# koide3/fast_gicp

Hardware: AMD Instinct MI355X
Metric: registrations/sec (100-iter reuse) + final fitness_score; achieved HBM GB/s (higher is better)
Workload: dtype f64

## Files before the change

### fast_gicp_amd/capi.py

```python
import ctypes as C
import os

import numpy as np

from . import build as _build

REG_NONE, REG_MIN_EIG, REG_NORMALIZED_MIN_EIG, REG_PLANE, REG_FROBENIUS = range(5)
DIRECT27, DIRECT7, DIRECT1, DIRECT_RADIUS = range(4)
NDT_P2D, NDT_D2D = 0, 1
COMPUTE_FP64, COMPUTE_FP32, COMPUTE_CUDA_COMPAT = 0, 1, 2
VOXEL_ADDITIVE, VOXEL_ADDITIVE_WEIGHTED, VOXEL_MULTIPLICATIVE = range(3)
VOXEL_NDT_SUMS = 3

EXPORTED_SYMBOLS = None


class LmParams(C.Structure):
    _fields_ = [("max_iterations", C.c_int), ("rotation_epsilon", C.c_double), ("transformation_epsilon", C.c_double), ("lm_max_iterations", C.c_int),
                ("lm_init_lambda_factor", C.c_double), ("optimizer", C.c_int)]


class LmResult(C.Structure):
    _fields_ = [("T", C.c_double * 16), ("H", C.c_double * 36), ("final_error", C.c_double), ("converged", C.c_int), ("nr_iterations", C.c_int),
                ("num_linearize", C.c_int), ("num_error_evals", C.c_int), ("lm_failed", C.c_int), ("num_launches", C.c_int)]


class EngineParams(C.Structure):
    _fields_ = [("struct_size", C.c_int), ("sort_mode", C.c_int), ("sort_items", C.c_int), ("sort_fused_bits", C.c_int), ("sort_two_pass_max", C.c_int),
                ("sort_coop_watchdog_ticks", C.c_ulonglong), ("knn_nearest_first_max_points", C.c_int), ("knn_block", C.c_int), ("coherent_min_points", C.c_int),
                ("bitmap_min_points", C.c_int), ("bitmap_max_bytes", C.c_ulonglong), ("persistent", C.c_int), ("persist_watchdog_ticks", C.c_ulonglong),
                ("peer_watchdog_ticks", C.c_ulonglong), ("lm_everywhere", C.c_int), ("cost_prio", C.c_int), ("cost_split", C.c_int), ("cost_group_max", C.c_int),
                ("cost_max_blocks", C.c_int), ("cost_target_items", C.c_longlong), ("zerocopy_result", C.c_int), ("host_wait_block", C.c_int),
                ("result_query_spins", C.c_ulonglong), ("side_stream", C.c_int), ("pinned_upload_max", C.c_ulonglong), ("zerocopy_upload_max", C.c_ulonglong),
                ("avg_fused", C.c_int), ("nn1_seed", C.c_int)]


def default_engine_params():
    p = EngineParams()
    load().fvh_default_engine_params(C.byref(p))
    return p


class FvhError(RuntimeError):
    pass


_LIB = None


# ... 356 lines not shown

def comm_unique_id():
    buf = (C.c_char * 128)()
    rc = load().fvh_comm_unique_id(buf)
    if rc != 0:
        raise FvhError("fvh_comm_unique_id failed: %d" % rc)
    return bytes(buf)


def debug_slot_pool(device=0):
    r, a, c = C.c_int(0), C.c_int(0), C.c_int(0)
    load().fvh_debug_slot_pool(int(device), C.byref(r), C.byref(a), C.byref(c))
    return r.value, a.value, c.value


def debug_sort_routes():
    a = (C.c_int * 4)()
    rc = load().fvh_debug_sort_routes(a)
    if rc != 0:
        raise FvhError("fvh_debug_sort_routes: status %d" % rc)
    return list(a)


def debug_xcd_local():
    w, a = C.c_int(0), C.c_int(0)
    load().fvh_debug_xcd_local(C.byref(w), C.byref(a))
    return w.value, a.value


LM_REPLAY_ARGTYPES = [C.c_int, C.c_void_p, C.c_void_p, C.c_int, C.c_void_p, C.c_void_p, C.c_void_p]
# ... 529 lines not shown
```

### fast_gicp_amd/csrc/fvh_capi.hip

```cpp
#include <hip/hip_runtime.h>
#include <dlfcn.h>

#include <algorithm>
#include <cmath>
#include <cstdio>
#include <cstdlib>
#include <atomic>
#include <chrono>
#include <cstring>
#include <functional>
#include <map>
#include <mutex>
#include <string>
#include <type_traits>
#include <unordered_map>
#include <vector>

#include "../../include/fast_vgicp_hip.h"
#include "kernels_compat.hpp"
#include "kernels_cost.hpp"
#include "kernels_cov.hpp"
#include "kernels_downsample.hpp"
#include "kernels_outlier.hpp"
#include "kernels_peer.hpp"
// ... 9 lines not shown
  int device = 0;
  fvh_engine_params params = env_engine_defaults();
  hipStream_t stream = nullptr;
  std::string err;
  int align_optimizer = 0;
  int precision = FVH_COMPUTE_FP64;
  bool float_cost() const { return precision != FVH_COMPUTE_FP64; }
  std::vector<int> offsets_host{0, 0, 0};
  int n_off = 1;
  DevBuf fit_best;
  DevBuf sort_coop;
  unsigned sort_seq = 0;
  DevBuf rbf_sums;
  bool abort_word_dirty = false;
  int last_persist_blocks = 0;
  bool zero_copy_armed = false;
  DevBuf bcast;
  unsigned long long persist_seq = 0;
  DevBuf offsets_dev, state, partials, ticket, corr, misc, fit, staging, sort_keys, sort_idx, sort_hist;
  void* pinned = nullptr;
  void* upload_pinned = nullptr;
  size_t upload_pinned_cap = 0;
  hipEvent_t upload_done[2] = {nullptr, nullptr};
  bool upload_busy[2] = {false, false};
  int upload_slot = 0;
  bool ensure_upload_pinned(size_t bytes) {
    if (bytes <= upload_pinned_cap) return true;
    for (int s = 0; s < 2; s++) {
      if (upload_busy[s]) { (void)hipEventSynchronize(upload_done[s]); upload_busy[s] = false; }
      if (!upload_done[s] && hipEventCreateWithFlags(&upload_done[s], hipEventDisableTiming) != hipSuccess) { (void)hipGetLastError(); return false; }
// ... 1040 lines not shown
}
int fvh_vgicp_set_lm_trace(fvh_vgicp* h, int on) { CHECK_HANDLE(h); return shared::set_lm_trace(h, on); }
int fvh_vgicp_get_lm_trace(fvh_vgicp* h, int* n, double* rows6) { CHECK_HANDLE(h); return shared::get_lm_trace(&h->e, n, rows6); }
int fvh_vgicp_fitness_score(fvh_vgicp* h, const double* T, double max_range, double* score) { CHECK_HANDLE(h); return do_fitness(&h->e, h->source, h->target, T, max_range, score); }
int fvh_vgicp_profile_enable(fvh_vgicp* h, int on) { CHECK_HANDLE_HOST_ONLY(h); return shared::profile_enable(h, on); }
int fvh_vgicp_profile_reset(fvh_vgicp* h) { CHECK_HANDLE(h); return shared::profile_reset(h); }
int fvh_vgicp_profile_get(fvh_vgicp* h, const char* cls, double* ms, int* n) { CHECK_HANDLE(h); return profile_get(&h->e, cls, ms, n); }
int fvh_vgicp_debug_set_voxel_hint(fvh_vgicp* h, int num_voxels) { CHECK_HANDLE(h); h->voxelmap.nv_hint = num_voxels; return FVH_OK; }
int fvh_vgicp_debug_get_persist_aborts(fvh_vgicp* h, int* n) { CHECK_HANDLE(h); if (!n) return FVH_ERR_INVALID_ARGUMENT; *n = h->e.persist_aborts; return FVH_OK; }
int fvh_vgicp_debug_get_persist_grid(fvh_vgicp* h, int* blocks, int* capacity) {
  CHECK_HANDLE(h);
  if (blocks) *blocks = h->e.last_persist_blocks;
  if (capacity) *capacity = persistent_capacity<MODE_VGICP>(&h->e);
  return FVH_OK;
}
int fvh_debug_sort_routes(int* counts4) {
  if (!counts4) return FVH_ERR_INVALID_ARGUMENT;
  for (int i = 0; i < 4; i++) counts4[i] = g_sort_routes[i].load();
  return FVH_OK;
}
int fvh_debug_xcd_local(int* wanted, int* placement_aborts) {
  if (wanted) *wanted = xcd_local_wanted() ? 1 : 0;
  if (placement_aborts) *placement_aborts = g_xcd_local_strikes.load();
  return FVH_OK;
}
int fvh_debug_slot_pool(int device, int* reserved, int* active, int* recent) {
  int r = 0, a = 0, c = 0;
  g_slots.snapshot(device, &r, &a, &c);
  if (reserved) *reserved = r;
  if (active) *active = a;
// ... 550 lines not shown
```

### fast_gicp_amd/csrc/host_runtime.inc.hpp

```cpp


constexpr int MAX_COST_BLOCKS = MAX_PARTIAL_ROWS;

struct DevBuf {
  void* p = nullptr;
  size_t cap = 0;
  hipError_t ensure(size_t bytes) {
    if (bytes <= cap) return hipSuccess;
    if (p) { hipError_t e = hipFree(p); p = nullptr; cap = 0; if (e != hipSuccess) return e; }
    size_t want = bytes + bytes / 4 + 256;
    hipError_t e = hipMalloc(&p, want);
    if (e == hipSuccess) cap = want;
    return e;
  }
  void release() { if (p) (void)hipFree(p); p = nullptr; cap = 0; }
  template <typename T> T* as() const { return reinterpret_cast<T*>(p); }
};

inline const char* fvh_env(const char* name) { return getenv(name); }
inline long long fvh_env_ll(const char* name, long long dflt) { const char* v = fvh_env(name); return v ? atoll(v) : dflt; }
inline unsigned long long fvh_env_ull(const char* name, unsigned long long dflt) { const char* v = fvh_env(name); return v ? strtoull(v, nullptr, 10) : dflt; }
constexpr int COHERENT_MIN_POINTS = 32768;
struct ProcessParams { int slot_max_split, contended_slot_pct, xcd_local, small_grid_layout; };
inline const ProcessParams& process_params() {
// ... 27 lines not shown
    p.peer_watchdog_ticks = fvh_env_ull("FVH_PEER_WATCHDOG_TICKS", 200'000'000ull);
    p.lm_everywhere = (int)fvh_env_ll("FVH_LM_EVERYWHERE", 1);
    { const char* v = fvh_env("FVH_COST_PRIO"); p.cost_prio = v ? (atoi(v) != 0 ? 1 : 0) : -1; }
    p.cost_split = (int)fvh_env_ll("FVH_COST_SPLIT", 1);
    p.cost_group_max = (int)std::min<long long>(std::max(1LL, fvh_env_ll("FVH_COST_GROUP_MAX", COST_CH)), COST_CH);
    { const long long b = fvh_env_ll("FVH_COST_MAX_BLOCKS", MAX_PARTIAL_ROWS); p.cost_max_blocks = (int)(b < 1 ? 1 : (b > MAX_PARTIAL_ROWS ? MAX_PARTIAL_ROWS : b)); }
    p.cost_target_items = fvh_env_ll("FVH_COST_TARGET_ITEMS", 256LL * 256 * 2);
    p.zerocopy_result = (int)fvh_env_ll("FVH_ZEROCOPY_RESULT", 1);
    { const char* v = fvh_env("FVH_HOST_WAIT"); p.host_wait_block = (v && std::string(v) == "block") ? 1 : 0; }
    p.result_query_spins = fvh_env_ull("FVH_RESULT_QUERY_SPINS", 1024ull);
    p.side_stream = fvh_env_ll("FVH_SIDE_STREAM", 1) != 0 ? 1 : 0;
    p.pinned_upload_max = fvh_env_ull("FVH_PINNED_UPLOAD_MAX", 8ull << 20);
    p.zerocopy_upload_max = fvh_env_ull("FVH_ZEROCOPY_UPLOAD_MAX", 1ull << 20);
    p.avg_fused = fvh_env_ll("FVH_AVG_FUSED", 1) != 0 ? 1 : 0;
    p.nn1_seed = fvh_env_ll("FVH_NN1_SEED", 1) != 0 ? 1 : 0;
    return p;
  }();
  return d;
}
inline const char* check_engine_params(const fvh_engine_params& p) {
  if (p.struct_size != (int)sizeof(fvh_engine_params)) return "engine params: struct_size does not match this library's fvh_engine_params (start from fvh_default_engine_params / fvh_*_get_engine_params)";
  if (p.sort_mode < 0 || p.sort_mode > 3) return "engine params: sort_mode must be 0..3";
  if (p.sort_fused_bits != 0 && p.sort_fused_bits != 9 && p.sort_fused_bits != 10) return "engine params: sort_fused_bits must be 0, 9 or 10";
  if (p.knn_block != 64 && p.knn_block != 128 && p.knn_block != 256) return "engine params: knn_block must be 64, 128 or 256";
  if (p.cost_group_max < 1 || p.cost_group_max > COST_CH) return "engine params: cost_group_max must be 1..4";
  if (p.cost_max_blocks < 1 || p.cost_max_blocks > MAX_PARTIAL_ROWS) return "engine params: cost_max_blocks must be 1..1024";
  if (p.cost_target_items < 1) return "engine params: cost_target_items must be positive";
  if (p.lm_everywhere < 0 || p.lm_everywhere > 2 || p.cost_prio < -1 || p.cost_prio > 1) return "engine params: lm_everywhere must be 0..2, cost_prio -1..1";
  if (p.bitmap_max_bytes > (16ull << 30)) return "engine params: bitmap_max_bytes beyond 16 GiB (the LM kernel indexes its words with 32 bits)";
  if (p.sort_items < 0 || p.sort_items > SORT_ITEMS_MAX || (p.sort_items & 63)) return "engine params: sort_items must be 0 or a multiple of 64 up to 1024";
  return nullptr;
}

struct CloudDev {
  int n = 0, k = 0;
  DevBuf box;
  DevBuf bbox2;
  DevBuf order;
  DevBuf pts, cov, nbr, bbox, sorted;
  bool has_pts = false, has_cov = false, has_nbr = false, has_sorted = false;
  DevBuf cov_sorted;
  bool has_cov_sorted = false;
  bool nbr_tile_only = false;
// ... 139 lines not shown
    reserved[dev] -= g.n;
    active[dev]--;
    if (recent[dev] > active[dev] + 1) {
      if (++calm[dev] >= DECAY_AFTER) { recent[dev]--; calm[dev] = 0; }
    } else {
      calm[dev] = 0;
    }
  }
};
SlotPool g_slots;
constexpr int XCD_LOCAL_MAX_STRIKES = 3;
std::atomic<int> g_xcd_local_strikes{0};
inline bool xcd_local_wanted() {
  return process_params().xcd_local && g_xcd_local_strikes.load() < XCD_LOCAL_MAX_STRIKES;
}
struct GridPlan { int nb = 0; int ng = 0; int local = 0; };
inline int small_grid_layout() {
  return process_params().small_grid_layout;
}
inline int default_groups(int nb) {
  if (nb > SINGLE_LEVEL_MAX_BLOCKS) return TICKET_GROUPS;
  return (small_grid_layout() == 2 && nb >= 2 * TICKET_GROUPS) ? TICKET_GROUPS : 1;
}
```

### fast_gicp_amd/csrc/host_stages.inc.hpp

```cpp

int upload_cloud(Engine* e, CloudDev& c, const float* xyz, int n, int stride, bool on_device, bool want_box = true ,
                 hipStream_t on = nullptr ) {
  hipStream_t const st = on ? on : e->stream;
  if (n < 0 || (n > 0 && !xyz)) return e->fail(FVH_ERR_INVALID_ARGUMENT, "set_cloud: null points");
  if (stride != 3 && stride != 4) return e->fail(FVH_ERR_INVALID_ARGUMENT, "set_cloud: stride must be 3 or 4 floats");
  HIP_OR_FAIL(e, c.pts.ensure(sizeof(float4) * (size_t)std::max(n, 1)));
  c.n = n;
  c.has_pts = true;
  c.has_sorted = false;
  if (n == 0) return FVH_OK;
  unsigned* boxp = nullptr;
  c.has_box = want_box;
  if (want_box) {
    const bool fresh_box = c.box.p == nullptr;
    HIP_OR_FAIL(e, c.box.ensure(64));
    if (fresh_box || c.box_dirty) HIP_OR_FAIL(e, hipMemsetAsync(c.box.p, 0, 64, st));
    c.box_dirty = true;
    boxp = c.box.as<unsigned>();
  }
  auto pack = [&](const float* srcp, int slot) -> int {
    pack_points_kernel<<<pack_grid(n, boxp != nullptr), 256, 0, st>>>(srcp, n, stride, c.pts.as<float4>(), boxp);
    HIP_OR_FAIL(e, hipGetLastError());
    if (slot >= 0) { HIP_OR_FAIL(e, hipEventRecord(e->upload_done[slot], st)); e->upload_busy[slot] = true; }
    return FVH_OK;
// ... 581 lines not shown
int persistent_capacity(Engine* e) {
  static std::mutex mu;
  static int cap[16][2];
  std::lock_guard<std::mutex> lk(mu);
  const int pi = e->float_cost() ? 1 : 0, dev = e->device & 15;
  if (cap[dev][pi] <= 0) {
    int per_cu = 0, cus = 0;
    hipError_t r = pi ? hipOccupancyMaxActiveBlocksPerMultiprocessor(&per_cu, cost_kernel<float, MODE, true>, 256, 0)
                      : hipOccupancyMaxActiveBlocksPerMultiprocessor(&per_cu, cost_kernel<double, MODE, true>, 256, 0);
    if (r != hipSuccess || hipDeviceGetAttribute(&cus, hipDeviceAttributeMultiprocessorCount, e->device) != hipSuccess) return 0;
    cap[dev][pi] = per_cu * cus;
  }
  return cap[dev][pi];
}

struct CostShape { int group, groups_per_src; long long n_walk; int blocks; int split; };
inline CostShape cost_shape(const Engine* e, const CostSource& src, int mode = MODE_VGICP, bool device_lm = false) {
  const long long target_items = e->params.cost_target_items;
  const int max_blocks = e->params.cost_max_blocks;
  const int group_max = e->params.cost_group_max;
  const int n_off = src.n_off_override > 0 ? src.n_off_override : e->n_off;
  CostShape s;
  const int n_expected = src.n_shape > 0 ? std::min(src.n_shape, src.n_upper) : src.n_upper;
  const int groups = (int)std::min<long long>(n_off, std::max<long long>((n_off + group_max - 1) / group_max, target_items / std::max(n_expected, 1)));
  s.group = (n_off + groups - 1) / groups;
  s.groups_per_src = (n_off + s.group - 1) / s.group;
  s.n_walk = n_expected;
  if (e->sharded() && src.shardable) { const Tile t = peer_tile(e, src.n_upper); s.n_walk = std::max(t.hi - t.lo, 0); }
  if (src.device_tile) s.n_walk = (n_expected + e->shard_ranks() - 1) / std::max(1, e->shard_ranks());
  s.blocks = (int)std::max<long long>(1, std::min<long long>(max_blocks, (s.n_walk * s.groups_per_src + 255) / 256));
// ... 73 lines not shown
    if (MODE == MODE_VGICP && e->peer.attached()) P.peer = e->peer.view(peer_xbase);
    P.peer_watchdog_ticks = e->params.peer_watchdog_ticks;
  }
  int blocks = shape.blocks;
  (void)n_walk;
  {
    int cap = persistent_capacity<MODE>(e);
    if (cap <= 0) return e->fail(FVH_ERR_HIP, "cost kernel: occupancy query failed");
    if (e->peer.attached()) cap = std::max(1, cap / std::max(1, e->peer.ranks_on_device));
    blocks = std::min(blocks, cap);
    if (plan && plan->nb > 0) blocks = std::min(blocks, plan->nb);
  }
  P.ng = (plan && plan->ng > 0) ? plan->ng : default_groups(blocks);
  if (P.ng > blocks) P.ng = 1;
  P.xcd_local = 0; P.lm_everywhere = 0;
  {
    const int prio = e->params.cost_prio;
    int cus = 256;
    (void)hipDeviceGetAttribute(&cus, hipDeviceAttributeMultiprocessorCount, e->device);
    P.prio_from = cus;
    P.prio_mode = prio >= 0 ? prio : ((persistent && blocks > cus && blocks <= 2 * cus) ? 1 : 0);
    const int everywhere = e->params.lm_everywhere;
    P.lm_everywhere = (persistent && P.ng > 1 && (everywhere == 2 || (everywhere == 1 && blocks <= 2 * cus))) ? 1 : 0;
  }
  if (persistent && plan) P.xcd_local = plan->local;
  GangParams G{blocks, nullptr};
  const int gangs = multi ? multi->k : 1;
  if (multi) {
    P.st = e->multi_state.as<LmState>(); P.partials = e->multi_partials.as<double>(); P.ticket = e->multi_ticket.as<unsigned>();
    P.bcast = e->multi_bcast.as<double>(); P.corr = e->multi_corr.as<int>(); P.lm_trace = nullptr;
    P.xcd_local = 0; P.prio_mode = 0;
    int cus = 256;
    (void)hipDeviceGetAttribute(&cus, hipDeviceAttributeMultiprocessorCount, e->device);
    P.lm_everywhere = (persistent && P.ng > 1 && (e->params.lm_everywhere == 2 || (e->params.lm_everywhere == 1 && (long long)gangs * blocks <= 2 * cus))) ? 1 : 0;
    G.guesses = e->multi_guess.as<PoseD>();
  }
  if (!multi && e->abort_word_dirty) {
    HIP_OR_FAIL(e, hipMemsetAsync(reinterpret_cast<char*>(e->state.p) + sizeof(LmState) - 8, 0, 8, e->stream));
    e->abort_word_dirty = false;
  }
  if (persistent) {
    P.watchdog_ticks = fvh_env_ull("FVH_PERSIST_WATCHDOG_TICKS", e->params.persist_watchdog_ticks);
    if (P.peer.n > 1 && P.watchdog_ticks) P.watchdog_ticks = std::max(P.watchdog_ticks, 2 * P.peer_watchdog_ticks);
    const int zc = e->params.zerocopy_result;
    P.result_host = (zc && (!e->prof.on || e->prof.cost_only)) ? (multi ? e->multi_result_dev : e->result_dev) : nullptr;
    e->zero_copy_armed = P.result_host != nullptr;
    if (!multi) P.bcast = e->bcast.as<double>();
    P.launch_tag = ++e->persist_seq;
    e->last_persist_blocks = blocks;
    (void)e->gang_begin(false);
  }
  {
    ProfScope ps(e, "cost");
    const bool gauss_newton = (host_phase < 0 ? e->align_optimizer : 0) != 0;
    by_flag(e->float_cost(), [&](auto f32) { by_flag(P.group == 1, [&](auto one) { by_flag(gauss_newton, [&](auto gn) { by_flag(persistent, [&](auto pers) {
      using Real = std::conditional_t<decltype(f32)::value, float, double>;
      constexpr int CH = decltype(one)::value ? 1 : COST_CH;
      if (multi) lm_gang_kernel<Real, MODE, decltype(pers)::value, CH, decltype(gn)::value><<<gangs * blocks, 256, 0, e->stream>>>(P, G);
      else cost_kernel<Real, MODE, decltype(pers)::value, CH, decltype(gn)::value><<<blocks, 256, 0, e->stream>>>(P);
    }); }); }); });
  }
  if (persistent) e->gang_end();
  HIP_OR_FAIL(e, hipGetLastError());
  return FVH_OK;
}

int allreduce_sums(Engine* e) {
  LmState* st = e->state.as<LmState>();
  int rc = g_rccl.AllReduce(st->sums, st->sums, PART_STRIDE,  8,  0, e->comm, e->stream);
  if (rc != 0) return e->fail(FVH_ERR_COMM, "ncclAllReduce failed with code " + std::to_string(rc));
  return FVH_OK;
}
// ... 146 lines not shown
  r->num_launches = (int)launches;
}

inline void leave_handle(Engine* e, const LmState& h, const fvh_lm_params& p, int corr_kind, int n_src) {
  e->prev_steps = e->last_steps;
  e->last_steps = p.optimizer ? std::max(1, (int)h.num_linearize) : 1 + h.num_error_evals;
  e->lin = h.x_lin;
  e->corr_sel = h.corr_cur;
  e->has_corr = true;
  e->corr_kind = corr_kind;
  e->corr_n_src = n_src;
}

template <int MODE>
int align_begin(Engine* e, AlignCtx& c, const CostSource& src, VoxelMapDev& vm, const double* guess16, const fvh_lm_params* params,
                bool retried = false, bool no_persist = false, const GridPlan* forced_plan = nullptr ) {
  hipEvent_t const fence = e->crowd_fence;
  e->crowd_fence = nullptr;
  e->lm_crowds_chip = false;
  if (!guess16) return e->fail(FVH_ERR_INVALID_ARGUMENT, "align: null argument");
  if (!vm.valid) return e->fail(FVH_ERR_BAD_STATE, "align: target voxel map not built");
  c = AlignCtx{};
  fvh_lm_params& p = c.p;
  if (params) p = *params; else fvh_default_lm_params(&p);
  std::memcpy(c.guess16, guess16, sizeof(c.guess16));
  e->align_optimizer = p.optimizer != 0 ? 1 : 0;
  c.retried = retried; c.no_persist = no_persist; c.grant_dev = e->device;
  HIP_OR_FAIL(e, e->corr.ensure(2 * sizeof(int) * (size_t)std::max(src.n_upper, 1) * e->n_off));
  const PoseD guess = pose_from_colmajor16(guess16);
  c.degenerate = p.max_iterations <= 0;
  if (c.degenerate) {
// ... 11 lines not shown
  if (c.persistent) {
    int cap = persistent_capacity<MODE>(e);
    if (e->peer.attached()) cap = std::max(1, cap / std::max(1, e->peer.ranks_on_device));
    const int want = std::min(cost_shape(e, src, MODE, true).blocks, std::max(cap, 1));
    const bool local_ok = xcd_local_wanted();
    c.grant = g_slots.acquire(e->device, std::max(cap, 1), want);
    int granted = c.grant.n;
    if (granted <= 0) {
      if (c.sharded) granted = want;
      else c.persistent = false;
    }
    c.plan = GridPlan{};
    c.plan.nb = granted;
    c.plan.ng = default_groups(granted);
    c.plan.local = (c.plan.ng == TICKET_GROUPS && local_ok) ? 1 : 0;
    e->lm_crowds_chip = c.persistent && Engine::crowds(c.plan.nb, std::max(cap, 1));
  }
  {
    if (c.persistent && e->lm_crowds_chip && fence && hipEventQuery(fence) != hipSuccess) {
      (void)hipGetLastError();
      HIP_OR_FAIL(e, hipStreamWaitEvent(e->stream, fence, 0));
    }
  }
  if (c.persistent) {
    int rc = launch_cost<MODE>(e, src, vm, -1, &guess, nullptr, &p, true, e->peer.x, &c.plan);
    if (rc) { c.release_slots(); return rc; }
  }
  c.active = true;
  return FVH_OK;
}
// ... 53 lines not shown
    fresh.refresh();
    return do_align<MODE>(e, fresh, vm, c.guess16, &p, result, rebuild_safe, true, no_persist, forced ? &plan : nullptr);
  }
  e->gang_clear();
  leave_handle(e, *h, p, 0 , src.n_upper);
  fill_result(*h, launched, result);
  e->lm_trace_rows = e->lm_trace_on ? h->num_error_evals : 0;
  return FVH_OK;
}

template <int MODE>
int do_align(Engine* e, const CostSource& src, VoxelMapDev& vm, const double* guess16, const fvh_lm_params* params, fvh_lm_result* result, const Rebuild& rebuild_safe,
             bool retried, bool no_persist, const GridPlan* forced_plan) {
  if (!result) return e->fail(FVH_ERR_INVALID_ARGUMENT, "align: null argument");
  AlignCtx c;
  int rc = align_begin<MODE>(e, c, src, vm, guess16, params, retried, no_persist, forced_plan);
  if (rc) return rc;
  return align_finish<MODE>(e, c, src, vm, result, rebuild_safe);
}

struct Pipeline {
  CloudDev next_source;
  VoxelMapDev next_map;
  bool next_ready = false;
  hipEvent_t prep_done = nullptr;
  AlignCtx pending;
  bool in_flight() const { return pending.active; }
  void invalidate() { next_map.invalidate(); next_ready = false; }
  void arm_crowd_fence(Engine* e) const { e->crowd_fence = next_ready ? prep_done : nullptr; }
  int begin_prepare(Engine* e, hipStream_t* ps) {
    if (e->side_stream() == nullptr && in_flight()) return e->fail(FVH_ERR_BAD_STATE, "prepare_source: this handle has no second stream; call it outside align_async .. align_wait");
// ... 221 lines not shown
```

### fast_gicp_amd/csrc/kernels_cost.hpp

```cpp
#pragma once
#include <cstddef>
#include <type_traits>

#include "dev_math.hpp"
#include "kernels_peer.hpp"
#include "kernels_voxelmap.hpp"

#pragma clang fp contract(on)

namespace fvh {

constexpr int NSUM = 28;
constexpr int PART_STRIDE = 32;
constexpr int MAX_PARTIAL_ROWS = 1024;

enum CostMode { MODE_VGICP = 0, MODE_NDT_P2D = 1, MODE_NDT_D2D = 2 };
enum Phase { PH_LINEARIZE = 0, PH_TRIAL = 1, PH_DONE = 2, PH_FIND_ONLY = 3, PH_EVAL_DERIV = 4, PH_EVAL_ERROR = 5,
             PH_TRIAL_FINAL = 6 };

struct LmState {
  PoseD x0;
  PoseD xi;
  PoseD x_lin;
  double H[36], b[6], d[6];
// ... 430 lines not shown
  for (int i = threadIdx.x; i < WORDS; i += 64) l[i] = g[i];
  __syncthreads();
  if (s.phase == PH_DONE) return;
  dev_lm_step_wave<GN>(&s, s.sums, threadIdx.x);
  __syncthreads();
  for (int i = threadIdx.x; i < WORDS; i += 64) g[i] = l[i];
}

template <typename Real>
struct ItemAcc {
  Sym3<Real> S;
  Vec3<Real> g;
  Real err;
};
template <typename Real>
__device__ __forceinline__ void hit_term(ItemAcc<Real>& it, const Vec3<Real>& q, const Vec3<Real>& mu, const Sym3<Real>& A, Real w, bool deriv) {
  const Vec3<Real> e = {mu.x - q.x, mu.y - q.y, mu.z - q.z};
  Real det;
  const Sym3<Real> C = adjugate(A, det);
  const Real s = fast_div(w, det);
  const Vec3<Real> Ce = mul(C, e);
  it.err += s * (e.x * Ce.x + e.y * Ce.y + e.z * Ce.z);
  if (!deriv) return;
  it.g.x += s * Ce.x; it.g.y += s * Ce.y; it.g.z += s * Ce.z;
  it.S.xx += s * C.xx; it.S.xy += s * C.xy; it.S.xz += s * C.xz; it.S.yy += s * C.yy; it.S.yz += s * C.yz; it.S.zz += s * C.zz;
}
template <typename Real>
__device__ __forceinline__ Real record_weight(const float4& q3) { return (Real)__hiloint2double(__float_as_int(q3.w), __float_as_int(q3.z)); }
template <typename Real>
__device__ __forceinline__ Real record_weight(const float2&) { return (Real)1; }
template <typename Real>
__device__ __forceinline__ void item_sums(double* v, const ItemAcc<Real>& it, const Vec3<Real>& q) {
  v[0] = (double)it.err;
  const Vec3<Real> bq = cross(it.g, q);
  v[1] = (double)bq.x; v[2] = (double)bq.y; v[3] = (double)bq.z;
// ... 127 lines not shown
  for (int k = 0; k < 9; k++) o.r[k] = p[which].r[k];
#pragma unroll
  for (int k = 0; k < 3; k++) o.t[k] = p[which].t[k];
  return o;
}

constexpr size_t GANG_TICKET_WORDS = 16;
constexpr size_t GANG_BCAST_DOUBLES = (size_t)PERSIST_REPLICAS * BCAST_PAIRS * 2;
constexpr size_t GANG_RESULT_WORDS = (sizeof(LmState) / 8 + 1 + 7) & ~(size_t)7;
constexpr int MAX_GANGS = 64;
struct GangParams {
  int nb_h;
  const PoseD* guesses;
};

template <typename Real, int MODE, bool PERSIST, int CH, bool GN, bool GANG>
__device__ __forceinline__ void cost_body(const CostParams& P, const unsigned gang_lb, const unsigned gang_nb, const unsigned gang, const PoseD* gang_guesses) {
  static_assert(CH == 1 || CH == COST_CH, "one or COST_CH lookups per item");
  auto lin_arg = [&]() -> PoseD { if constexpr (GANG) return gang_guesses[gang]; else return P.lin; };
  auto partials = [&]() -> double* { if constexpr (GANG) return P.partials + (size_t)gang * PARTIALS_DOUBLES; else return P.partials; };
  auto ticket = [&]() -> unsigned* { if constexpr (GANG) return P.ticket + (size_t)gang * GANG_TICKET_WORDS; else return P.ticket; };
  auto bcast_base = [&]() -> double* { if constexpr (GANG) return P.bcast + (size_t)gang * GANG_BCAST_DOUBLES; else return P.bcast; };
  auto corr_base = [&]() -> int* { if constexpr (GANG) return P.corr + (size_t)gang * 2 * P.corr_stride; else return P.corr; };
  auto result_host = [&]() -> unsigned long long* { if constexpr (GANG) return P.result_host ? P.result_host + (size_t)gang * GANG_RESULT_WORDS : nullptr; else return P.result_host; };
#ifdef FVH_COST_TIMING
  __shared__ unsigned long long stamp[12];
  if (threadIdx.x == 0) { stamp[0] = wall_clock64(); atomicMin(&g_cost_timing[0], stamp[0]); }
#endif
  __shared__ double red[4][PART_STRIDE];
  __shared__ double fin[8][PART_STRIDE];
  __shared__ int s_last;
  __shared__ LmState s_st;
  static_assert(sizeof(LmState) % 8 == 0, "LmState is copied as 64-bit words");
// ... 32 lines not shown
  if (threadIdx.x < 8) {
    const int t = threadIdx.x;
    int gv = 0, rv = 0;
    if (P.bitmap && P.grid) gv = t < 3 ? P.grid->b0[t] : (t < 6 ? P.grid->nb[t - 3] : (t == 6 ? P.grid->enabled : 0));
    if (P.region) rv = t < 3 ? P.region->inner_lo[t] : (t < 6 ? P.region->inner_hi[t - 3] : 0);
    s_grid[t] = gv; s_region[t] = rv;
  }
  __syncthreads();
  const int n_src_launch = P.d_n_src ? *P.d_n_src : P.n_src;
  constexpr int STICKY_T = PERSIST ? 256 : 1;
  __shared__ float4 s_src[3][STICKY_T];
  constexpr int ELEM_ITS = 2;
  __shared__ int s_elem[PERSIST ? ELEM_ITS : 1][STICKY_T];
  __shared__ int s_ids[2][CH][STICKY_T];
  __shared__ int s_ofp[CH][STICKY_T];
  bool a_primed = false;
  for (;;) {
  if (PERSIST) FVH_PT_MIN(gen, 0);
  const bool fused = (P.host_phase < 0) && (phase == PH_TRIAL);
  constexpr bool EXT_OK = !PERSIST && MODE == MODE_VGICP;
  const bool external = EXT_OK && P.external_find != 0;
  const bool do_find = !external && ((phase == PH_LINEARIZE) || (phase == PH_FIND_ONLY) || fused);
  const bool do_cost = (phase != PH_FIND_ONLY);
  const bool do_deriv = (phase == PH_LINEARIZE) || (phase == PH_EVAL_DERIV) || fused;
  const Real res = (Real)P.res, inv_res = (Real)P.inv_res;
  const int n_src = n_src_launch;
  int w_lo = (P.item_hi > 0 ? min(P.item_lo, n_src) : 0) * P.groups_per_src;
  int n_items = (P.item_hi > 0 ? min(P.item_hi, n_src) : n_src) * P.groups_per_src;
  if (P.tile_n > 1) {
    const int chunk = (n_src + P.tile_n - 1) / P.tile_n, lo = min(P.tile_rank * chunk, n_src);
    w_lo = lo * P.groups_per_src;
    n_items = min(lo + chunk, n_src) * P.groups_per_src;
  }
  int* corr_old = corr_base() + (size_t)corr_sel * P.corr_stride;
  int* corr_new = fused ? corr_base() + (size_t)(corr_sel ^ 1) * P.corr_stride : corr_old;
  constexpr bool SPLIT_OK = (MODE != MODE_VGICP) && CH == 1;
  const bool split = SPLIT_OK && P.split != 0;
  const int wave_id = __builtin_amdgcn_readfirstlane((int)(threadIdx.x >> 6));
  const bool role_a = split && wave_id < 2;
  const bool role_b = split && wave_id >= 2;
  const int wstride = split ? 128 : 256;
  const bool sticky = PERSIST && ((long long)(n_items - w_lo) <= (long long)nb * wstride);
  const bool cached = sticky && (role_a ? a_primed : gen > 0);
  const int sel_new = fused ? (corr_sel ^ 1) : corr_sel;

  double wacc = 0.0;
  const int lane = threadIdx.x & 63;

  const float4* tf = reinterpret_cast<const float4*>(P.table);
  int item_no = -1;
  for (int wbase = w_lo + (int)lb * wstride + (split ? ((wave_id & 1) << 6) : (int)(threadIdx.x & 192)); wbase < n_items; wbase += (int)nb * wstride) {
    item_no++;
    if (role_a && !fused) continue;
    const int w = wbase + lane;
    ItemAcc<Real> it = {{0, 0, 0, 0, 0, 0}, {0, 0, 0}, 0};
    Real acc_y = 0;
    if (PERSIST && P.prio_mode && lb >= (unsigned)P.prio_from) __builtin_amdgcn_s_setprio(1);
    Vec3<Real> q = {0, 0, 0};
    bool any_hit = false;
// ... 95 lines not shown
        Vec3<Real> ql = q;
        if (!fused) { const Pose<Real> lin = lds_pose(pose_ptr, 0); ql = transform(lin, a); }
        const Real fx = floor(div_by(ql.x, res, inv_res) - (Real)0.5), fy = floor(div_by(ql.y, res, inv_res) - (Real)0.5), fz = floor(div_by(ql.z, res, inv_res) - (Real)0.5);
        coord_ok = voxel_index_ok(fx, fy, fz);
        cx = coord_ok ? (int)fx : 0;
        cy = coord_ok ? (int)fy : 0;
        cz = coord_ok ? (int)fz : 0;
        if (P.region) {
          LdsInt rg = (LdsInt)s_region;
          asm volatile("" : "+v"(rg));
          const int l0 = rg[0], l1 = rg[1], l2 = rg[2], h0 = rg[3], h1 = rg[4], h2 = rg[5];
          left_shard = coord_ok && ((cx < l0) | (cx > h0) | (cy < l1) | (cy > h1) | (cz < l2) | (cz > h2));
        }
      }
    }
    if (MODE != MODE_NDT_P2D && do_cost) {
      const Sym3<Real> CA = {(Real)c0.x, (Real)c0.y, (Real)c0.z, (Real)c0.w, (Real)c1.x, (Real)c1.y};
      Real Rl[9];
#pragma unroll
      for (int k = 0; k < 9; k++) Rl[k] = pose_ptr[0].r[k];
      if (fused) { if (!role_b) RCR_old = rotate_cov(Rl, CA); } else RCR = rotate_cov(Rl, CA);
    }
    if (PERSIST) FVH_MT(gen, 2);
    {
      unsigned long long key[CH];
      unsigned slot[CH];
      unsigned long long k0[CH];
      float4 sq1 = make_float4(0, 0, 0, 0), sq2 = sq1;
      Q3 sq3 = {};
      constexpr unsigned long long DEAD_KEY = FVH_EMPTY_KEY - 1;
      if (do_find && !role_a) {
// ... 31 lines not shown
          }
        }
#pragma unroll
        for (int c = 0; c < CH; c++) {
          slot[c] = hash_slot(key[c], P.mask);
          k0[c] = P.keys[(filtered && !live[c]) ? 0u : slot[c]];
        }
        if constexpr (CH == 1) {
          if (do_cost && !(fused && (int)slot[0] == bo[0])) {
            const size_t sb = (size_t)slot[0] * 4;
            sq1 = tf[sb + 1]; sq2 = tf[sb + 2]; sq3 = *reinterpret_cast<const Q3*>(tf + sb + 3);
          }
        }
      }
      if (PERSIST) FVH_MT(gen, 3);
      if (fused && do_cost && !role_b) {
#pragma unroll
        for (int c = 0; c < CH; c++) {
          if (bo[c] < 0) continue;
          const float4 o1 = q1[c], o2 = q2[c];
          const Q3 o3 = q3[c];
          const int npts = (int)o1.w;
          const Vec3<Real> mu = {(Real)o1.x, (Real)o1.y, (Real)o1.z};
          const Sym3<Real> A = {(Real)o2.x + RCR_old.xx, (Real)o2.y + RCR_old.xy, (Real)o2.z + RCR_old.xz, (Real)o2.w + RCR_old.yy, (Real)o3.x + RCR_old.yz, (Real)o3.y + RCR_old.zz};
          const Vec3<Real> e = {mu.x - q.x, mu.y - q.y, mu.z - q.z};
          Real wgt;
          if constexpr (MODE == MODE_VGICP) {
            if (npts <= 0) continue;
            wgt = record_weight<Real>(o3);
          } else {
            if (npts <= 6) continue;
// ... 52 lines not shown
      for (int c = 0; c < CH; c++) {
        if (b[c] < 0) continue;
        const int npts = (int)q1[c].w;
        const Vec3<Real> mu = {(Real)q1[c].x, (Real)q1[c].y, (Real)q1[c].z};
        const Sym3<Real> A = {(Real)q2[c].x + RCR.xx, (Real)q2[c].y + RCR.xy, (Real)q2[c].z + RCR.xz, (Real)q2[c].w + RCR.yy, (Real)q3[c].x + RCR.yz, (Real)q3[c].y + RCR.zz};
        Real wgt;
        if constexpr (MODE == MODE_VGICP) {
          if (npts <= 0) continue;
          wgt = record_weight<Real>(q3[c]);
        } else {
          if (npts <= 6) continue;
          const Real ex = mu.x - q.x, ey = mu.y - q.y, ez = mu.z - q.z;
          const Real ksq = res * res;
          wgt = ksq / (ksq + (ex * ex + ey * ey + ez * ez));
        }
        hit_term<Real>(it, q, mu, A, wgt, do_deriv);
        any_hit = true;
      }
      }
    }
    }
    if (PERSIST && P.prio_mode) __builtin_amdgcn_s_setprio(0);
    if (!do_cost) continue;
    if (PERSIST) FVH_MT(gen, 7);
    if (role_a) {
      double tot = (double)acc_y;
#pragma unroll
      for (int off = 32; off > 0; off >>= 1) tot += __shfl_xor(tot, off);
      if ((lane >> 1) == NSUM) wacc += tot;
      continue;
    }
// ... 23 lines not shown
        for (int j = 0; j < 4; j++) {
          if (j < half) {
            const double lo = v[j], hi = v[j + half];
            const double recv = __shfl_xor(up ? lo : hi, m);
            v[j] = (up ? hi : lo) + recv;
          }
        }
      }
      v[0] += __shfl_xor(v[0], 1);
      wacc += v[0];
    }
    if (PERSIST) FVH_MT(gen, 8);
  }

  if (role_a && fused) a_primed = true;
  if (!do_cost) return;
  int tid = threadIdx.x;
  asm volatile("" : "+v"(tid));
  FVH_STAMP(1);
  if (PERSIST) FVH_PT_MAX(gen, 1);
  if ((tid & 1) == 0) red[tid >> 6][(tid & 63) >> 1] = wacc;
  __syncthreads();

  const unsigned NG = (unsigned)P.ng;
  const unsigned grp = lb % NG;
  const unsigned ngroups = NG;
  const unsigned gsize = (nb - grp + NG - 1) / NG;
  if constexpr (!PERSIST) {
    if (tid < PART_STRIDE) {
      const int vv = tid;
// ... 367 lines not shown
    if (tid < 24) {
      const int which = tid / 12, k = tid % 12;
      const Real v = (Real)bc[2 + tid];
      if (k < 9) s_pose[which].r[k] = v; else s_pose[which].t[k - 9] = v;
    }
    __syncthreads();
  }
  }
}

template <typename Real, int MODE, bool PERSIST, int CH = COST_CH, bool GN = false>
__global__ FVH_COST_BOUNDS void cost_kernel(CostParams P) {
  cost_body<Real, MODE, PERSIST, CH, GN, false>(P, 0u, 0u, 0u, nullptr);
}

template <typename Real, int MODE, bool PERSIST, int CH = COST_CH, bool GN = false>
__global__ FVH_COST_BOUNDS void lm_gang_kernel(CostParams P, GangParams G) {
  const unsigned nb_h = (unsigned)G.nb_h;
  const unsigned gang = blockIdx.x / nb_h;
  cost_body<Real, MODE, PERSIST, CH, GN, true>(P, blockIdx.x - gang * nb_h, nb_h, gang, G.guesses);
}

}
```

### include/fast_vgicp_hip.h

```cpp
#ifndef FAST_VGICP_HIP_H
#define FAST_VGICP_HIP_H

#ifdef __cplusplus
extern "C" {
#endif

typedef struct fvh_vgicp fvh_vgicp;
typedef struct fvh_ndt fvh_ndt;

enum fvh_status { FVH_OK = 0, FVH_ERR_INVALID_ARGUMENT = 1, FVH_ERR_BAD_STATE = 2, FVH_ERR_HIP = 3, FVH_ERR_UNSUPPORTED = 4, FVH_ERR_COMM = 5 };

enum fvh_regularization { FVH_REG_NONE = 0, FVH_REG_MIN_EIG = 1, FVH_REG_NORMALIZED_MIN_EIG = 2, FVH_REG_PLANE = 3, FVH_REG_FROBENIUS = 4 };
enum fvh_neighbor_search { FVH_DIRECT27 = 0, FVH_DIRECT7 = 1, FVH_DIRECT1 = 2, FVH_DIRECT_RADIUS = 3 };
enum fvh_ndt_distance_mode { FVH_NDT_P2D = 0, FVH_NDT_D2D = 1 };
enum fvh_precision { FVH_COMPUTE_FP64 = 0, FVH_COMPUTE_FP32 = 1, FVH_COMPUTE_CUDA_COMPAT = 2 };

typedef struct fvh_lm_params {
  int max_iterations;
  double rotation_epsilon;
  double transformation_epsilon;
  int lm_max_iterations;
  double lm_init_lambda_factor;
  int optimizer;
} fvh_lm_params;
// ... 30 lines not shown
  unsigned long long peer_watchdog_ticks;
  int lm_everywhere;
  int cost_prio;
  int cost_split;
  int cost_group_max;
  int cost_max_blocks;
  long long cost_target_items;
  int zerocopy_result;
  int host_wait_block;
  unsigned long long result_query_spins;
  int side_stream;
  unsigned long long pinned_upload_max;
  unsigned long long zerocopy_upload_max;
  int avg_fused;
  int nn1_seed;
} fvh_engine_params;
void fvh_default_engine_params(fvh_engine_params* p);

int fvh_vgicp_create(int device, fvh_vgicp** out);
int fvh_vgicp_destroy(fvh_vgicp* h);
const char* fvh_vgicp_last_error(const fvh_vgicp* h);

int fvh_vgicp_set_resolution(fvh_vgicp* h, double resolution);
int fvh_vgicp_set_kernel_params(fvh_vgicp* h, double kernel_width, double kernel_max_dist);
int fvh_vgicp_set_neighbor_search_method(fvh_vgicp* h, int method, double radius);
int fvh_vgicp_set_precision(fvh_vgicp* h, int precision);
int fvh_vgicp_get_engine_params(fvh_vgicp* h, fvh_engine_params* out);
int fvh_vgicp_set_engine_params(fvh_vgicp* h, const fvh_engine_params* p);
enum fvh_voxel_accumulation_mode { FVH_VOXEL_ADDITIVE = 0, FVH_VOXEL_ADDITIVE_WEIGHTED = 1, FVH_VOXEL_MULTIPLICATIVE = 2 };
enum { FVH_VOXEL_NDT_SUMS = 3 };
// ... 63 lines not shown
int fvh_vgicp_gicp_swap_source_and_target(fvh_vgicp* h);
int fvh_vgicp_gicp_update_correspondences(fvh_vgicp* h, const double* T16);
int fvh_vgicp_gicp_compute_error(fvh_vgicp* h, const double* T16, double* H36, double* b6, double* error);
int fvh_vgicp_gicp_align(fvh_vgicp* h, const double* guess16, const fvh_lm_params* params, fvh_lm_result* result);
int fvh_vgicp_gicp_get_correspondences(fvh_vgicp* h, int* target_index_per_source_point );

int fvh_vgicp_profile_enable(fvh_vgicp* h, int on );
int fvh_vgicp_profile_reset(fvh_vgicp* h);
int fvh_vgicp_profile_get(fvh_vgicp* h, const char* kernel_class, double* total_ms, int* launches);
int fvh_vgicp_synchronize(fvh_vgicp* h);
int fvh_vgicp_debug_set_voxel_hint(fvh_vgicp* h, int num_voxels);
int fvh_vgicp_debug_get_table_capacity(fvh_vgicp* h, int* capacity);
int fvh_vgicp_debug_get_skipped_points(fvh_vgicp* h, int* n);
int fvh_vgicp_debug_get_persist_aborts(fvh_vgicp* h, int* n);
int fvh_vgicp_debug_get_persist_grid(fvh_vgicp* h, int* blocks, int* capacity);
int fvh_debug_slot_pool(int device, int* reserved, int* active, int* recent);
#define FVH_LM_REPLAY_ROW 133
int fvh_debug_lm_replay(int device, const double* guess16, const fvh_lm_params* params, int n_steps, const double* sums ,
                        double* rows , int* steps_run);
int fvh_debug_regularize(int device, int n, const double* sym6, int method, double* w3, double* V9, double* reg6);
int fvh_debug_xcd_local(int* wanted, int* placement_aborts);
int fvh_debug_sort_routes(int* counts4);

int fvh_comm_unique_id(void* id128 );
int fvh_vgicp_comm_init(fvh_vgicp* h, const void* id128, int nranks, int rank);
int fvh_vgicp_comm_destroy(fvh_vgicp* h);

int fvh_vgicp_peer_export(fvh_vgicp* h, int max_points, void* ipc_handle64 , unsigned long long* process_local_ptr );
int fvh_vgicp_peer_attach(fvh_vgicp* h, int nranks, int rank, int ranks_on_this_device, const void* ipc_handles ,
                          const unsigned long long* process_local_ptrs );
// ... 107 lines not shown
```

Measured before the change: 5373.

## Carry per-thread adjugate terms across LM trial evaluations in a sticky persistent kernel

Adds a specialized persistent Levenberg-Marquardt kernel variant that keeps each thread's covariance adjugate and scale in registers after a linearization. Later error-only trial evaluations on the same correspondence set reuse them instead of reloading covariances, rotating them and recomputing the adjugate. With the default setting it is enabled only when the align runs alone on the device, the work fits in one item per thread, and the grid fits occupancy. This trades extra register pressure (launch bounds 256,2) and a new code path for less arithmetic and memory traffic per trial.

```diff
diff --git a/fast_gicp_amd/capi.py b/fast_gicp_amd/capi.py
--- a/fast_gicp_amd/capi.py
+++ b/fast_gicp_amd/capi.py
@@ -32,7 +32,7 @@
                 ("peer_watchdog_ticks", C.c_ulonglong), ("lm_everywhere", C.c_int), ("cost_prio", C.c_int), ("cost_split", C.c_int), ("cost_group_max", C.c_int),
                 ("cost_max_blocks", C.c_int), ("cost_target_items", C.c_longlong), ("zerocopy_result", C.c_int), ("host_wait_block", C.c_int),
                 ("result_query_spins", C.c_ulonglong), ("side_stream", C.c_int), ("pinned_upload_max", C.c_ulonglong), ("zerocopy_upload_max", C.c_ulonglong),
-                ("avg_fused", C.c_int), ("nn1_seed", C.c_int)]
+                ("avg_fused", C.c_int), ("nn1_seed", C.c_int), ("lm_carry", C.c_int)]
 
 
 def default_engine_params():
@@ -419,6 +419,12 @@
     return r.value, a.value, c.value
 
 
+def debug_lm_kernel_sticky(core):
+    n = C.c_int(0)
+    core._call("debug_get_lm_kernel", C.byref(n))
+    return n.value
+
+
 def debug_sort_routes():
     a = (C.c_int * 4)()
     rc = load().fvh_debug_sort_routes(a)
diff --git a/fast_gicp_amd/csrc/fvh_capi.hip b/fast_gicp_amd/csrc/fvh_capi.hip
--- a/fast_gicp_amd/csrc/fvh_capi.hip
+++ b/fast_gicp_amd/csrc/fvh_capi.hip
@@ -47,6 +47,7 @@
   DevBuf rbf_sums;
   bool abort_word_dirty = false;
   int last_persist_blocks = 0;
+  int last_persist_sticky = 0;
   bool zero_copy_armed = false;
   DevBuf bcast;
   unsigned long long persist_seq = 0;
@@ -1117,6 +1118,7 @@
   if (capacity) *capacity = persistent_capacity<MODE_VGICP>(&h->e);
   return FVH_OK;
 }
+int fvh_vgicp_debug_get_lm_kernel(fvh_vgicp* h, int* sticky) { CHECK_HANDLE(h); if (!sticky) return FVH_ERR_INVALID_ARGUMENT; *sticky = h->e.last_persist_sticky; return FVH_OK; }
 int fvh_debug_sort_routes(int* counts4) {
   if (!counts4) return FVH_ERR_INVALID_ARGUMENT;
   for (int i = 0; i < 4; i++) counts4[i] = g_sort_routes[i].load();
diff --git a/fast_gicp_amd/csrc/host_runtime.inc.hpp b/fast_gicp_amd/csrc/host_runtime.inc.hpp
--- a/fast_gicp_amd/csrc/host_runtime.inc.hpp
+++ b/fast_gicp_amd/csrc/host_runtime.inc.hpp
@@ -65,6 +65,7 @@
     p.zerocopy_upload_max = fvh_env_ull("FVH_ZEROCOPY_UPLOAD_MAX", 1ull << 20);
     p.avg_fused = fvh_env_ll("FVH_AVG_FUSED", 1) != 0 ? 1 : 0;
     p.nn1_seed = fvh_env_ll("FVH_NN1_SEED", 1) != 0 ? 1 : 0;
+    { const long long v = fvh_env_ll("FVH_LM_CARRY", -1); p.lm_carry = v < 0 ? -1 : (v > 0 ? 1 : 0); }
     return p;
   }();
   return d;
@@ -78,6 +79,7 @@
   if (p.cost_max_blocks < 1 || p.cost_max_blocks > MAX_PARTIAL_ROWS) return "engine params: cost_max_blocks must be 1..1024";
   if (p.cost_target_items < 1) return "engine params: cost_target_items must be positive";
   if (p.lm_everywhere < 0 || p.lm_everywhere > 2 || p.cost_prio < -1 || p.cost_prio > 1) return "engine params: lm_everywhere must be 0..2, cost_prio -1..1";
+  if (p.lm_carry < -1 || p.lm_carry > 1) return "engine params: lm_carry must be -1..1";
   if (p.bitmap_max_bytes > (16ull << 30)) return "engine params: bitmap_max_bytes beyond 16 GiB (the LM kernel indexes its words with 32 bits)";
   if (p.sort_items < 0 || p.sort_items > SORT_ITEMS_MAX || (p.sort_items & 63)) return "engine params: sort_items must be 0 or a multiple of 64 up to 1024";
   return nullptr;
@@ -247,7 +249,7 @@
 inline bool xcd_local_wanted() {
   return process_params().xcd_local && g_xcd_local_strikes.load() < XCD_LOCAL_MAX_STRIKES;
 }
-struct GridPlan { int nb = 0; int ng = 0; int local = 0; };
+struct GridPlan { int nb = 0; int ng = 0; int local = 0; int alone = 0; };
 inline int small_grid_layout() {
   return process_params().small_grid_layout;
 }
diff --git a/fast_gicp_amd/csrc/host_stages.inc.hpp b/fast_gicp_amd/csrc/host_stages.inc.hpp
--- a/fast_gicp_amd/csrc/host_stages.inc.hpp
+++ b/fast_gicp_amd/csrc/host_stages.inc.hpp
@@ -619,6 +619,23 @@
   return cap[dev][pi];
 }
 
+inline int sticky_capacity(Engine* e, bool one_lookup) {
+  static std::mutex mu;
+  static int cap[16][2][2];
+  std::lock_guard<std::mutex> lk(mu);
+  const int pi = e->float_cost() ? 1 : 0, ci = one_lookup ? 1 : 0, dev = e->device & 15;
+  if (cap[dev][pi][ci] <= 0) {
+    int per_cu = 0, cus = 0;
+    hipError_t r = pi ? (ci ? hipOccupancyMaxActiveBlocksPerMultiprocessor(&per_cu, lm_sticky_kernel<float, MODE_VGICP, 1>, 256, 0)
+                            : hipOccupancyMaxActiveBlocksPerMultiprocessor(&per_cu, lm_sticky_kernel<float, MODE_VGICP, COST_CH>, 256, 0))
+                      : (ci ? hipOccupancyMaxActiveBlocksPerMultiprocessor(&per_cu, lm_sticky_kernel<double, MODE_VGICP, 1>, 256, 0)
+                            : hipOccupancyMaxActiveBlocksPerMultiprocessor(&per_cu, lm_sticky_kernel<double, MODE_VGICP, COST_CH>, 256, 0));
+    if (r != hipSuccess || hipDeviceGetAttribute(&cus, hipDeviceAttributeMultiprocessorCount, e->device) != hipSuccess) return 0;
+    cap[dev][pi][ci] = per_cu * cus;
+  }
+  return cap[dev][pi][ci];
+}
+
 struct CostShape { int group, groups_per_src; long long n_walk; int blocks; int split; };
 inline CostShape cost_shape(const Engine* e, const CostSource& src, int mode = MODE_VGICP, bool device_lm = false) {
   const long long target_items = e->params.cost_target_items;
@@ -722,6 +739,7 @@
   P.ng = (plan && plan->ng > 0) ? plan->ng : default_groups(blocks);
   if (P.ng > blocks) P.ng = 1;
   P.xcd_local = 0; P.lm_everywhere = 0;
+  bool sticky_kernel = false;
   {
     const int prio = e->params.cost_prio;
     int cus = 256;
@@ -730,6 +748,12 @@
     P.prio_mode = prio >= 0 ? prio : ((persistent && blocks > cus && blocks <= 2 * cus) ? 1 : 0);
     const int everywhere = e->params.lm_everywhere;
     P.lm_everywhere = (persistent && P.ng > 1 && (everywhere == 2 || (everywhere == 1 && blocks <= 2 * cus))) ? 1 : 0;
+    const int carry = e->params.lm_carry;
+    if (MODE == MODE_VGICP && persistent && host_phase < 0 && carry != 0 && !multi && !src.d_n && !e->sharded() && !e->peer.attached() && e->align_optimizer == 0) {
+      const long long items = (long long)src.n_upper * shape.groups_per_src;
+      const bool legal = items <= (long long)blocks * 256 && blocks <= 2 * cus && blocks <= sticky_capacity(e, P.group == 1);
+      sticky_kernel = legal && (carry == 1 || (plan && plan->alone));
+    }
   }
   if (persistent && plan) P.xcd_local = plan->local;
   GangParams G{blocks, nullptr};
@@ -756,6 +780,7 @@
     if (!multi) P.bcast = e->bcast.as<double>();
     P.launch_tag = ++e->persist_seq;
     e->last_persist_blocks = blocks;
+    e->last_persist_sticky = sticky_kernel ? 1 : 0;
     (void)e->gang_begin(false);
   }
   {
@@ -764,6 +789,9 @@
     by_flag(e->float_cost(), [&](auto f32) { by_flag(P.group == 1, [&](auto one) { by_flag(gauss_newton, [&](auto gn) { by_flag(persistent, [&](auto pers) {
       using Real = std::conditional_t<decltype(f32)::value, float, double>;
       constexpr int CH = decltype(one)::value ? 1 : COST_CH;
+      if constexpr (MODE == MODE_VGICP && decltype(pers)::value && !decltype(gn)::value) {
+        if (sticky_kernel) { lm_sticky_kernel<Real, MODE_VGICP, CH><<<blocks, 256, 0, e->stream>>>(P); return; }
+      }
       if (multi) lm_gang_kernel<Real, MODE, decltype(pers)::value, CH, decltype(gn)::value><<<gangs * blocks, 256, 0, e->stream>>>(P, G);
       else cost_kernel<Real, MODE, decltype(pers)::value, CH, decltype(gn)::value><<<blocks, 256, 0, e->stream>>>(P);
     }); }); }); });
@@ -940,7 +968,8 @@
 
 template <int MODE>
 int align_begin(Engine* e, AlignCtx& c, const CostSource& src, VoxelMapDev& vm, const double* guess16, const fvh_lm_params* params,
-                bool retried = false, bool no_persist = false, const GridPlan* forced_plan = nullptr ) {
+                bool retried = false, bool no_persist = false, const GridPlan* forced_plan = nullptr ,
+                bool blocking = false ) {
   hipEvent_t const fence = e->crowd_fence;
   e->crowd_fence = nullptr;
   e->lm_crowds_chip = false;
@@ -982,6 +1011,11 @@
     c.plan.nb = granted;
     c.plan.ng = default_groups(granted);
     c.plan.local = (c.plan.ng == TICKET_GROUPS && local_ok) ? 1 : 0;
+    if (blocking && c.grant.n > 0) {
+      int reserved = 0, active = 0, recent = 0;
+      g_slots.snapshot(e->device, &reserved, &active, &recent);
+      c.plan.alone = (active == 1 && reserved == c.grant.n) ? 1 : 0;
+    }
     e->lm_crowds_chip = c.persistent && Engine::crowds(c.plan.nb, std::max(cap, 1));
   }
   {
@@ -1065,7 +1099,7 @@
              bool retried, bool no_persist, const GridPlan* forced_plan) {
   if (!result) return e->fail(FVH_ERR_INVALID_ARGUMENT, "align: null argument");
   AlignCtx c;
-  int rc = align_begin<MODE>(e, c, src, vm, guess16, params, retried, no_persist, forced_plan);
+  int rc = align_begin<MODE>(e, c, src, vm, guess16, params, retried, no_persist, forced_plan, true);
   if (rc) return rc;
   return align_finish<MODE>(e, c, src, vm, result, rebuild_safe);
 }
diff --git a/fast_gicp_amd/csrc/kernels_cost.hpp b/fast_gicp_amd/csrc/kernels_cost.hpp
--- a/fast_gicp_amd/csrc/kernels_cost.hpp
+++ b/fast_gicp_amd/csrc/kernels_cost.hpp
@@ -468,11 +468,13 @@
   Real err;
 };
 template <typename Real>
-__device__ __forceinline__ void hit_term(ItemAcc<Real>& it, const Vec3<Real>& q, const Vec3<Real>& mu, const Sym3<Real>& A, Real w, bool deriv) {
+__device__ __forceinline__ void hit_term(ItemAcc<Real>& it, const Vec3<Real>& q, const Vec3<Real>& mu, const Sym3<Real>& A, Real w, bool deriv,
+                                         Sym3<Real>* keep_adj = nullptr, Real* keep_s = nullptr) {
   const Vec3<Real> e = {mu.x - q.x, mu.y - q.y, mu.z - q.z};
   Real det;
   const Sym3<Real> C = adjugate(A, det);
   const Real s = fast_div(w, det);
+  if (keep_adj) { *keep_adj = C; *keep_s = s; }
   const Vec3<Real> Ce = mul(C, e);
   it.err += s * (e.x * Ce.x + e.y * Ce.y + e.z * Ce.z);
   if (!deriv) return;
@@ -630,9 +632,10 @@
   const PoseD* guesses;
 };
 
-template <typename Real, int MODE, bool PERSIST, int CH, bool GN, bool GANG>
+template <typename Real, int MODE, bool PERSIST, int CH, bool GN, bool GANG, bool CARRY = false>
 __device__ __forceinline__ void cost_body(const CostParams& P, const unsigned gang_lb, const unsigned gang_nb, const unsigned gang, const PoseD* gang_guesses) {
   static_assert(CH == 1 || CH == COST_CH, "one or COST_CH lookups per item");
+  static_assert(!CARRY || (MODE == MODE_VGICP && PERSIST && !GN && !GANG), "carried terms: the persistent Levenberg-Marquardt VGICP kernel of a single align");
   auto lin_arg = [&]() -> PoseD { if constexpr (GANG) return gang_guesses[gang]; else return P.lin; };
   auto partials = [&]() -> double* { if constexpr (GANG) return P.partials + (size_t)gang * PARTIALS_DOUBLES; else return P.partials; };
   auto ticket = [&]() -> unsigned* { if constexpr (GANG) return P.ticket + (size_t)gang * GANG_TICKET_WORDS; else return P.ticket; };
@@ -695,6 +698,14 @@
   __shared__ int s_elem[PERSIST ? ELEM_ITS : 1][STICKY_T];
   __shared__ int s_ids[2][CH][STICKY_T];
   __shared__ int s_ofp[CH][STICKY_T];
+  constexpr int KEEP_N = CARRY ? CH : 1;
+  Sym3<Real> keep_adj[KEEP_N];
+  Real keep_s[KEEP_N];
+  int keep_sel = -1;
+  if constexpr (CARRY) {
+#pragma unroll
+    for (int c = 0; c < KEEP_N; c++) { keep_adj[c] = {0, 0, 0, 0, 0, 0}; keep_s[c] = 0; }
+  }
   bool a_primed = false;
   for (;;) {
   if (PERSIST) FVH_PT_MIN(gen, 0);
@@ -724,6 +735,7 @@
   const bool sticky = PERSIST && ((long long)(n_items - w_lo) <= (long long)nb * wstride);
   const bool cached = sticky && (role_a ? a_primed : gen > 0);
   const int sel_new = fused ? (corr_sel ^ 1) : corr_sel;
+  const bool kept = CARRY && sticky && fused && keep_sel == corr_sel;
 
   double wacc = 0.0;
   const int lane = threadIdx.x & 63;
@@ -849,7 +861,7 @@
         }
       }
     }
-    if (MODE != MODE_NDT_P2D && do_cost) {
+    if (MODE != MODE_NDT_P2D && do_cost && !kept) {
       const Sym3<Real> CA = {(Real)c0.x, (Real)c0.y, (Real)c0.z, (Real)c0.w, (Real)c1.x, (Real)c1.y};
       Real Rl[9];
 #pragma unroll
@@ -911,7 +923,18 @@
         }
       }
       if (PERSIST) FVH_MT(gen, 3);
-      if (fused && do_cost && !role_b) {
+      if (CARRY && kept) {
+#pragma unroll
+        for (int c = 0; c < KEEP_N; c++) {
+          if (bo[c] < 0) continue;
+          const float4 o1 = q1[c];
+          if ((int)o1.w <= 0) continue;
+          const Vec3<Real> mu = {(Real)o1.x, (Real)o1.y, (Real)o1.z};
+          const Vec3<Real> e = {mu.x - q.x, mu.y - q.y, mu.z - q.z};
+          const Vec3<Real> Ce = mul(keep_adj[c], e);
+          acc_y += keep_s[c] * (e.x * Ce.x + e.y * Ce.y + e.z * Ce.z);
+        }
+      } else if (fused && do_cost && !role_b) {
 #pragma unroll
         for (int c = 0; c < CH; c++) {
           if (bo[c] < 0) continue;
@@ -994,7 +1017,8 @@
           const Real ksq = res * res;
           wgt = ksq / (ksq + (ex * ex + ey * ey + ez * ez));
         }
-        hit_term<Real>(it, q, mu, A, wgt, do_deriv);
+        if constexpr (CARRY) hit_term<Real>(it, q, mu, A, wgt, do_deriv, &keep_adj[c], &keep_s[c]);
+        else hit_term<Real>(it, q, mu, A, wgt, do_deriv);
         any_hit = true;
       }
       }
@@ -1048,6 +1072,7 @@
   }
 
   if (role_a && fused) a_primed = true;
+  if constexpr (CARRY) keep_sel = sel_new;
   if (!do_cost) return;
   int tid = threadIdx.x;
   asm volatile("" : "+v"(tid));
@@ -1445,6 +1470,11 @@
   cost_body<Real, MODE, PERSIST, CH, GN, false>(P, 0u, 0u, 0u, nullptr);
 }
 
+template <typename Real, int MODE, int CH = COST_CH>
+__global__ __launch_bounds__(256, 2) void lm_sticky_kernel(CostParams P) {
+  cost_body<Real, MODE, true, CH, false, false, true>(P, 0u, 0u, 0u, nullptr);
+}
+
 template <typename Real, int MODE, bool PERSIST, int CH = COST_CH, bool GN = false>
 __global__ FVH_COST_BOUNDS void lm_gang_kernel(CostParams P, GangParams G) {
   const unsigned nb_h = (unsigned)G.nb_h;
diff --git a/include/fast_vgicp_hip.h b/include/fast_vgicp_hip.h
--- a/include/fast_vgicp_hip.h
+++ b/include/fast_vgicp_hip.h
@@ -68,6 +68,7 @@
   unsigned long long zerocopy_upload_max;
   int avg_fused;
   int nn1_seed;
+  int lm_carry;
 } fvh_engine_params;
 void fvh_default_engine_params(fvh_engine_params* p);
 
@@ -161,6 +162,7 @@
 int fvh_vgicp_debug_get_skipped_points(fvh_vgicp* h, int* n);
 int fvh_vgicp_debug_get_persist_aborts(fvh_vgicp* h, int* n);
 int fvh_vgicp_debug_get_persist_grid(fvh_vgicp* h, int* blocks, int* capacity);
+int fvh_vgicp_debug_get_lm_kernel(fvh_vgicp* h, int* sticky);
 int fvh_debug_slot_pool(int device, int* reserved, int* active, int* recent);
 #define FVH_LM_REPLAY_ROW 133
 int fvh_debug_lm_replay(int device, const double* guess16, const fvh_lm_params* params, int n_steps, const double* sums ,
```

After: 5525, median of 6. 1.03x the previous value.
